# codelion/adaptive-classifier

Measured on NVIDIA H100. Metric: queries/sec predict() bert-base 128-tok, 1M x 768 prototypes, higher is better.
Workload: dtype f16

## Files before the change

### adaptive_classifier_b200/csrc/api.cu

```cuda
#include "common.cuh"
#include <cstdarg>
#include <cudaTypedefs.h>
#include <atomic>
#include <mutex>
#include <vector>

namespace ac {

static thread_local char g_err[512] = "";

void set_error(const char *fmt, ...) {
    va_list ap;
    va_start(ap, fmt);
    vsnprintf(g_err, sizeof(g_err), fmt, ap);
    va_end(ap);
}

int check_cuda(cudaError_t e, const char *what) {
    if (e == cudaSuccess) return AC_OK;
    set_error("CUDA error %d (%s) at %s", static_cast<int>(e), cudaGetErrorString(e), what);
    return AC_E_CUDA;
}

static std::atomic<long long> g_launches{0};
void count_launch() { g_launches.fetch_add(1, std::memory_order_relaxed); }
void count_launch_n(long long n) { g_launches.fetch_add(n, std::memory_order_relaxed); }
long long launch_count_now() { return g_launches.load(std::memory_order_relaxed); }

struct ProfSlot { cudaEvent_t a, b; int cls; double flops, bytes; };
static bool g_prof_on = false;
bool prof_is_on() { return g_prof_on; }
static std::vector<ProfSlot> g_prof_slots;
static size_t g_prof_used = 0;
static double g_prof_ms[PROF_NUM], g_prof_flops[PROF_NUM], g_prof_bytes[PROF_NUM];
static long long g_prof_n[PROF_NUM];

static void prof_harvest() {
    cudaDeviceSynchronize();
    for (size_t i = 0; i < g_prof_used; ++i) {
        float ms = 0.f;
        if (cudaEventElapsedTime(&ms, g_prof_slots[i].a, g_prof_slots[i].b) == cudaSuccess) {
            const int c = g_prof_slots[i].cls;
            g_prof_ms[c] += ms; g_prof_flops[c] += g_prof_slots[i].flops; g_prof_bytes[c] += g_prof_slots[i].bytes;
            g_prof_n[c] += 1;
        }
    }
    g_prof_used = 0;
}

int prof_begin(int cls, double flops, double bytes, cudaStream_t s) {
    if (!g_prof_on) return -1;
    if (g_prof_used == g_prof_slots.size()) {
        if (g_prof_slots.size() >= 8192) {
            prof_harvest();
        } else {
            ProfSlot p{};
            if (cudaEventCreate(&p.a) != cudaSuccess || cudaEventCreate(&p.b) != cudaSuccess) return -1;
            g_prof_slots.push_back(p);
        }
    }
    ProfSlot &p = g_prof_slots[g_prof_used];
    p.cls = cls; p.flops = flops; p.bytes = bytes;
    cudaEventRecord(p.a, s);
    return static_cast<int>(g_prof_used++);
}
void prof_end(int slot, cudaStream_t s) {
    if (slot < 0) return;
    cudaEventRecord(g_prof_slots[slot].b, s);
}

int sm_count() {
    static int n = 0;
    if (n == 0) {
        int dev = 0;
        if (cudaGetDevice(&dev) != cudaSuccess) return 132;
        if (cudaDeviceGetAttribute(&n, cudaDevAttrMultiProcessorCount, dev) != cudaSuccess || n <= 0) n = 132;
    }
    return n;
}

int make_tmap_2d(CUtensorMap *out, const void *gptr, int elem_bytes, uint64_t rows, uint64_t cols,
                 uint64_t row_stride_bytes, uint32_t box_rows, uint32_t box_cols) {
    static PFN_cuTensorMapEncodeTiled_v12000 encode = nullptr;
    static std::once_flag once;
    std::call_once(once, [] {
        void *fn = nullptr;
        cudaDriverEntryPointQueryResult qres;
        if (cudaGetDriverEntryPoint("cuTensorMapEncodeTiled", &fn, cudaEnableDefault, &qres) == cudaSuccess &&
            qres == cudaDriverEntryPointSuccess)
            encode = reinterpret_cast<PFN_cuTensorMapEncodeTiled_v12000>(fn);
    });
    if (!encode) {
        set_error("cuTensorMapEncodeTiled entry point not available (no CUDA driver?)");
        return AC_E_CUDA;
    }
    AC_REQUIRE((reinterpret_cast<uintptr_t>(gptr) & 15) == 0 && row_stride_bytes % 16 == 0,
               "make_tmap_2d: base pointer and row stride must be 16-byte aligned");
    AC_REQUIRE(box_cols * static_cast<uint32_t>(elem_bytes) == 128 && box_rows <= 256,
               "make_tmap_2d: box must be 128 bytes wide and <= 256 rows");
    const CUtensorMapDataType dt = (elem_bytes == 4) ? CU_TENSOR_MAP_DATA_TYPE_FLOAT32 : CU_TENSOR_MAP_DATA_TYPE_FLOAT16;
    cuuint64_t gdim[2] = {cols, rows};
    cuuint64_t gstride[1] = {row_stride_bytes};
    cuuint32_t box[2] = {box_cols, box_rows};
    cuuint32_t estr[2] = {1, 1};
    CUresult r = encode(out, dt, 2, const_cast<void *>(gptr), gdim, gstride, box, estr, CU_TENSOR_MAP_INTERLEAVE_NONE,
                        CU_TENSOR_MAP_SWIZZLE_128B, CU_TENSOR_MAP_L2_PROMOTION_L2_256B,
                        CU_TENSOR_MAP_FLOAT_OOB_FILL_NONE);
    if (r != CUDA_SUCCESS) {
        set_error("cuTensorMapEncodeTiled failed with CUresult %d (rows=%llu cols=%llu)", static_cast<int>(r),
                  static_cast<unsigned long long>(rows), static_cast<unsigned long long>(cols));
        return AC_E_CUDA;
    }
    return AC_OK;
}

int launch_knn_dist_exact(const float *Q, const float *P, int nq, int64_t N, int D, float *Dout, cudaStream_t stream);
int launch_knn_rerank(const float *Q, const float *P, int B, int64_t N, int D, int kc, const int32_t *cand, float *out_d,
                      int64_t *out_i, int64_t row_offset, cudaStream_t stream);
size_t topk_select_workspace(int B, int64_t L, int k);
int topk_select(const float *d, const int64_t *idx, int B, int64_t L, int64_t in_stride, int64_t id_offset, int k,
                float *out_d, int64_t *out_i, void *ws, size_t ws_bytes, cudaStream_t stream, const float *row_gate = nullptr);
size_t knn_tc_workspace(int B, int64_t N, int D, int k);
int knn_tc_search(const float *Q, const float *P, const float *p_sqnorm, const void *p_half, int B, int64_t N, int D, int k,
                  float *out_d, int64_t *out_i, int64_t row_offset, void *ws, size_t ws_bytes, int32_t *stats, cudaStream_t stream);

static int exact_query_block(int B, int64_t N) {
    const int64_t budget = 256ll << 20;
    int64_t qb = budget / (4 * (N > 0 ? N : 1));
    if (qb < 1) qb = 1;
    if (qb > B) qb = B;
    if (qb > 64) qb = 64;
    return static_cast<int>(qb);
}

static size_t knn_exact_workspace(int B, int64_t N, int k) {
    const int qb = exact_query_block(B, N);
    return align_up(static_cast<size_t>(qb) * N * sizeof(float), 256) + topk_select_workspace(qb, N, k) + 256;
}

static int knn_exact(const float *Q, const float *P, int B, int64_t N, int D, int k, float *out_d, int64_t *out_i,
                     int64_t row_offset, void *ws, size_t ws_bytes, cudaStream_t s) {
    const int qb = exact_query_block(B, N);
    const size_t dist_bytes = align_up(static_cast<size_t>(qb) * N * sizeof(float), 256);
    if (dist_bytes > ws_bytes) { set_error("ac_knn_l2_topk: workspace too small"); return AC_E_WORKSPACE; }
    float *dist = static_cast<float *>(ws);
    uint8_t *sel_ws = static_cast<uint8_t *>(ws) + dist_bytes;
    const size_t sel_bytes = ws_bytes - dist_bytes;
    for (int b0 = 0; b0 < B; b0 += qb) {
        const int nb = (B - b0 < qb) ? B - b0 : qb;
        int rc = launch_knn_dist_exact(Q + static_cast<int64_t>(b0) * D, P, nb, N, D, dist, s);
        if (rc) return rc;
        rc = topk_select(dist, nullptr, nb, N, N, row_offset, k, out_d + static_cast<int64_t>(b0) * k,
                         out_i + static_cast<int64_t>(b0) * k, sel_ws, sel_bytes, s);
        if (rc) return rc;
    }
    return AC_OK;
}

static int resolve_algo(int algo, int B, int64_t N, int D, int k) {
    if (algo != AC_KNN_AUTO) return algo;
    if (B >= 16 && k <= AC_KNN_TENSOR_MAX_K && N >= 4096 && N >= 8ll * k && D % 32 == 0) return AC_KNN_TENSOR;
    return AC_KNN_EXACT;
}

}

using namespace ac;

extern "C" int ac_version(void) { return 1; }
extern "C" long long ac_launch_count(void) { return g_launches.load(); }
extern "C" int ac_profile_enable(int on) {
    if (on && !g_prof_on) {
        for (int c = 0; c < PROF_NUM; ++c) { g_prof_ms[c] = g_prof_flops[c] = g_prof_bytes[c] = 0; g_prof_n[c] = 0; }
        g_prof_used = 0;
    }
    if (!on && g_prof_on) prof_harvest();
    g_prof_on = on != 0;
    return AC_OK;
}
extern "C" int ac_profile_read(int cls, double *ms, double *flops, double *bytes, long long *launches) {
    AC_REQUIRE(cls >= 0 && cls < PROF_NUM, "ac_profile_read: bad class");
    prof_harvest();
    if (ms) *ms = g_prof_ms[cls];
    if (flops) *flops = g_prof_flops[cls];
    if (bytes) *bytes = g_prof_bytes[cls];
    if (launches) *launches = g_prof_n[cls];
    return AC_OK;
}
extern "C" const char *ac_last_error(void) { return g_err; }

extern "C" int ac_device_check(void) {
    int n = 0;
    cudaError_t e = cudaGetDeviceCount(&n);
    if (e != cudaSuccess || n <= 0) {
        set_error("no CUDA device visible (%s); this library has no CPU fallback", cudaGetErrorString(e));
        return AC_E_CUDA;
    }
    int dev = 0, major = 0, minor = 0;
    AC_CUDA(cudaGetDevice(&dev));
    AC_CUDA(cudaDeviceGetAttribute(&major, cudaDevAttrComputeCapabilityMajor, dev));
    AC_CUDA(cudaDeviceGetAttribute(&minor, cudaDevAttrComputeCapabilityMinor, dev));
    if (major != 9 || minor != 0) {
        set_error("device compute capability %d.%d is not sm_90 (H100); kernels are sm_90a only", major, minor);
        return AC_E_CUDA;
    }
    return AC_OK;
}

extern "C" int ac_knn_workspace_bytes(int B, int64_t N, int D, int k, int algo, size_t *bytes) {
    AC_REQUIRE(bytes && B >= 0 && N >= 0 && D > 0 && k >= 1, "ac_knn_workspace_bytes: bad arguments");
    AC_REQUIRE(k <= AC_KNN_MAX_K, "ac_knn_workspace_bytes: k=%d > %d", k, AC_KNN_MAX_K);
    const int a = resolve_algo(algo, B, N, D, k);
    size_t need = knn_exact_workspace(B, N, k);
    if (a == AC_KNN_TENSOR) need += knn_tc_workspace(B, N, D, k);
    *bytes = need + 256;
    return AC_OK;
}

extern "C" int ac_knn_l2_topk(const float *Q, const float *P, const float *p_sqnorm, const void *p_half, int B, int64_t N,
                              int D, int k, float *out_d, int64_t *out_i, int64_t row_offset, void *workspace,
                              size_t workspace_bytes, int algo, int32_t *stats, ac_stream_t stream) {
    AC_REQUIRE(Q && out_d && out_i && B >= 0 && N >= 0 && D > 0, "ac_knn_l2_topk: bad arguments");
    AC_REQUIRE(k >= 1 && k <= AC_KNN_MAX_K, "ac_knn_l2_topk: k=%d outside [1,%d]", k, AC_KNN_MAX_K);
    AC_REQUIRE(N == 0 || P, "ac_knn_l2_topk: null index");
    AC_REQUIRE(N < (1ll << 31), "ac_knn_l2_topk: shards are limited to 2^31-1 rows");
    if (B == 0) return AC_OK;
    cudaStream_t s = static_cast<cudaStream_t>(stream);
    const int a = resolve_algo(algo, B, N, D, k);
    uint8_t *ws = static_cast<uint8_t *>(workspace);
    ws = reinterpret_cast<uint8_t *>(align_up(reinterpret_cast<uintptr_t>(ws), 256));
    const size_t slack = static_cast<size_t>(ws - static_cast<uint8_t *>(workspace));
    AC_REQUIRE(workspace && workspace_bytes > slack, "ac_knn_l2_topk: null/empty workspace");
    const size_t avail = workspace_bytes - slack;
    if (a == AC_KNN_TENSOR) {
        AC_REQUIRE(k <= AC_KNN_TENSOR_MAX_K && D % 32 == 0, "ac_knn_l2_topk: tensor path needs k <= %d and D %% 32 == 0", AC_KNN_TENSOR_MAX_K);
        AC_REQUIRE(!p_half || D % 64 == 0, "ac_knn_l2_topk: the fp16 shadow path needs D %% 64 == 0");
        return knn_tc_search(Q, P, p_sqnorm, p_half, B, N, D, k, out_d, out_i, row_offset, ws, avail, stats, s);
    }
    return knn_exact(Q, P, B, N, D, k, out_d, out_i, row_offset, ws, avail, s);
}

namespace ac {
int knn_exact_subset(const float *Q, const float *P, int B, int64_t N, int D, int k, float *out_d, int64_t *out_i,
                     int64_t row_offset, void *ws, size_t ws_bytes, cudaStream_t s) {
    return knn_exact(Q, P, B, N, D, k, out_d, out_i, row_offset, ws, ws_bytes, s);
}
size_t knn_exact_workspace_pub(int B, int64_t N, int k) { return knn_exact_workspace(B, N, k); }
}
```

### adaptive_classifier_b200/csrc/gemm_tc.cuh

```cuda
#pragma once
#include "common.cuh"

namespace ac {

constexpr int GEMM_BLOCK_M = 128;
constexpr int GEMM_BLOCK_N = 128;
constexpr int GEMM_BLOCK_K = 32;
constexpr int GEMM_KIND_TF32 = 0, GEMM_KIND_F16 = 1;
__host__ __device__ constexpr int gemm_block_k(int kind) { return kind == GEMM_KIND_F16 ? 64 : 32; }
constexpr int GEMM_STAGES = 4;
constexpr int GEMM_EPI_COLS = GEMM_BLOCK_N / 2;
constexpr int GEMM_EPI_WARPS = 8;
constexpr int GEMM_MMA_THREAD0 = 32 * GEMM_EPI_WARPS;
constexpr int GEMM_PRODUCER_THREAD = GEMM_MMA_THREAD0 + 128;
constexpr int GEMM_THREADS = GEMM_PRODUCER_THREAD + 128;
constexpr int GEMM_EPI_REGS = 160, GEMM_MMA_REGS = 160, GEMM_PRODUCER_REGS = 24;
static_assert(128 * GEMM_PRODUCER_REGS + 128 * GEMM_MMA_REGS + 256 * GEMM_EPI_REGS <= 65536, "register split exceeds the file");
constexpr int GEMM_A_STAGE_BYTES = GEMM_BLOCK_M * 128;
constexpr int GEMM_B_STAGE_BYTES = GEMM_BLOCK_N * 128;
constexpr int GEMM_STAGE_BYTES = GEMM_A_STAGE_BYTES + GEMM_B_STAGE_BYTES;
constexpr int GEMM_ACC_LD = GEMM_BLOCK_N + 4;
constexpr int GEMM_ACC_BYTES = GEMM_BLOCK_M * GEMM_ACC_LD * 4;
constexpr int GEMM_EPI_STAGE_ROW_BYTES = 80;
constexpr int GEMM_EPI_STAGE_BYTES = 32 * GEMM_EPI_STAGE_ROW_BYTES;
constexpr int GEMM_SMEM_BYTES = GEMM_STAGES * GEMM_STAGE_BYTES + GEMM_ACC_BYTES + GEMM_EPI_WARPS * GEMM_EPI_STAGE_BYTES +
                                1024  + 256 ;
static_assert(GEMM_SMEM_BYTES <= 227 * 1024, "stage ring + accumulator tile do not fit");

#ifndef AC_MBAR_WATCHDOG
#define AC_MBAR_WATCHDOG 1
#endif

__device__ __forceinline__ void mbar_wait_guarded(uint64_t *bar, uint32_t parity) {
#if AC_MBAR_WATCHDOG
    uint32_t spins = 0;
    while (!mbar_try_wait(bar, parity)) {
        if (++spins > (1u << 26)) __trap();
    }
#else
    mbar_wait(bar, parity);
#endif
}

struct GemmTileInfo {
    int m0, n0;
    int tile_iter;
};

__device__ __forceinline__ int gemm_epi_chalf() { return ((threadIdx.x >> 5) >> 1) & 1; }

template <class Epi, bool kMFastest = false, int kKind = GEMM_KIND_TF32>
__global__ void __launch_bounds__(GEMM_THREADS, 1)
gemm_tc_kernel(const __grid_constant__ CUtensorMap tmap_a, const __grid_constant__ CUtensorMap tmap_b,
               int M, int N, int K, Epi epi) {
    if (epi.skip_kernel()) return;
    extern __shared__ uint8_t smem_raw[];
    uint8_t *smem = reinterpret_cast<uint8_t *>((reinterpret_cast<uintptr_t>(smem_raw) + 1023) & ~uintptr_t(1023));
    uint8_t *smem_a = smem;
    uint8_t *smem_b = smem + GEMM_STAGES * GEMM_A_STAGE_BYTES;
    float *acc_tile = reinterpret_cast<float *>(smem + GEMM_STAGES * GEMM_STAGE_BYTES);
    uint8_t *epi_stage = smem + GEMM_STAGES * GEMM_STAGE_BYTES + GEMM_ACC_BYTES;
    uint64_t *bars = reinterpret_cast<uint64_t *>(epi_stage + GEMM_EPI_WARPS * GEMM_EPI_STAGE_BYTES);
    uint64_t *full_bar = bars;
    uint64_t *empty_bar = bars + GEMM_STAGES;
    uint64_t *acc_full = bars + 2 * GEMM_STAGES;
    uint64_t *acc_empty = acc_full + 1;

    const int warp = threadIdx.x >> 5;
    const int lane = threadIdx.x & 31;
    const int tiles_m = (M + GEMM_BLOCK_M - 1) / GEMM_BLOCK_M;
    const int tiles_n = (N + GEMM_BLOCK_N - 1) / GEMM_BLOCK_N;
    const int num_tiles = tiles_m * tiles_n;
    constexpr int BK = gemm_block_k(kKind);
    const int num_kb = (K + BK - 1) / BK;
    const int my_tiles = (num_tiles - static_cast<int>(blockIdx.x) + static_cast<int>(gridDim.x) - 1) / static_cast<int>(gridDim.x);

    if (threadIdx.x == GEMM_PRODUCER_THREAD) {
        tma_prefetch_desc(&tmap_a);
        tma_prefetch_desc(&tmap_b);
        for (int s = 0; s < GEMM_STAGES; ++s) {
            mbar_init(&full_bar[s], 1);
            mbar_init(&empty_bar[s], 4);
        }
        mbar_init(acc_full, 128);
        mbar_init(acc_empty, 32 * GEMM_EPI_WARPS);
        fence_mbar_init();
    }
    __syncthreads();

    if (threadIdx.x >= GEMM_PRODUCER_THREAD) {
        setmaxnreg_dec<GEMM_PRODUCER_REGS>();
        if (threadIdx.x == GEMM_PRODUCER_THREAD) {
            int stage = 0;
            uint32_t phase = 0;
            for (int tile = blockIdx.x; tile < num_tiles; tile += gridDim.x) {
                const int m0 = (kMFastest ? tile % tiles_m : tile / tiles_n) * GEMM_BLOCK_M;
                const int n0 = (kMFastest ? tile / tiles_m : tile % tiles_n) * GEMM_BLOCK_N;
                for (int kb = 0; kb < num_kb; ++kb) {
                    mbar_wait_guarded(&empty_bar[stage], phase ^ 1);
                    mbar_arrive_expect_tx(&full_bar[stage], GEMM_STAGE_BYTES);
                    tma_load_2d(smem_a + stage * GEMM_A_STAGE_BYTES, &tmap_a, &full_bar[stage], kb * BK, m0);
                    tma_load_2d(smem_b + stage * GEMM_B_STAGE_BYTES, &tmap_b, &full_bar[stage], kb * BK, n0);
                    if (++stage == GEMM_STAGES) { stage = 0; phase ^= 1; }
                }
            }
        }
        return;
    }

    if (threadIdx.x >= GEMM_MMA_THREAD0) {
        setmaxnreg_inc<GEMM_MMA_REGS>();
        const uint64_t a_desc0 = wgmma_desc_sw128(smem_u32(smem_a));
        const uint64_t b_desc0 = wgmma_desc_sw128(smem_u32(smem_b));
        int stage = 0;
        uint32_t phase = 0;
        for (int it = 0; it < my_tiles; ++it) {
            float acc0[64], acc1[64];
#pragma unroll
            for (int j = 0; j < 64; ++j) { acc0[j] = 0.f; acc1[j] = 0.f; }
            int prev_stage = -1;
            for (int kb = 0; kb < num_kb; ++kb) {
                mbar_wait_guarded(&full_bar[stage], phase);
                const uint64_t a_desc = a_desc0 + stage * (GEMM_A_STAGE_BYTES >> 4);
                const uint64_t b_desc = b_desc0 + stage * (GEMM_B_STAGE_BYTES >> 4);
                wgmma_fence();
#pragma unroll
                for (int k = 0; k < 4; ++k) {
                    if (kKind == GEMM_KIND_F16) {
                        wgmma_m64n128_f16(acc0, a_desc + 2 * k, b_desc + 2 * k, 1u);
                        wgmma_m64n128_f16(acc1, a_desc + 512 + 2 * k, b_desc + 2 * k, 1u);
                    } else {
                        wgmma_m64n128_tf32(acc0, a_desc + 2 * k, b_desc + 2 * k, 1u);
                        wgmma_m64n128_tf32(acc1, a_desc + 512 + 2 * k, b_desc + 2 * k, 1u);
                    }
                }
                wgmma_commit();
                wgmma_wait<1>();
                __syncwarp();
                if (prev_stage >= 0 && lane == 0) mbar_arrive(&empty_bar[prev_stage]);
                prev_stage = stage;
                if (++stage == GEMM_STAGES) { stage = 0; phase ^= 1; }
            }
            wgmma_wait<0>();
            __syncwarp();
            if (lane == 0) mbar_arrive(&empty_bar[prev_stage]);

            mbar_wait_guarded(acc_empty, (it & 1) ^ 1);
            wgmma_store_acc(acc0, acc_tile, GEMM_ACC_LD);
            wgmma_store_acc(acc1, acc_tile + 64 * GEMM_ACC_LD, GEMM_ACC_LD);
            mbar_arrive(acc_full);
        }
        return;
    }

    setmaxnreg_inc<GEMM_EPI_REGS>();
    const int wg = warp >> 2;
    const int q = 2 * wg + (warp & 1);
    const int chalf = gemm_epi_chalf();
    typename Epi::State est;
    epi.begin_cta(est, q, lane);
    const float *acc_row = acc_tile + (q * 32 + lane) * GEMM_ACC_LD;
    for (int it = 0; it < my_tiles; ++it) {
        const int tile = static_cast<int>(blockIdx.x) + it * static_cast<int>(gridDim.x);
        GemmTileInfo ti;
        ti.m0 = (kMFastest ? tile % tiles_m : tile / tiles_n) * GEMM_BLOCK_M;
        ti.n0 = (kMFastest ? tile / tiles_m : tile % tiles_n) * GEMM_BLOCK_N;
        ti.tile_iter = it;
        const int row = ti.m0 + q * 32 + lane;
        const int c_lo = chalf * GEMM_EPI_COLS;
        constexpr int kDist = Epi::kPrefetchDist, kBufs = kDist + 1, kChunks = GEMM_EPI_COLS / 32;
#pragma unroll
        for (int d = 0; d < kDist; ++d)
            if (d < kChunks) epi.prefetch(est, ti, row, ti.n0 + c_lo + 32 * d, lane, d % kBufs);

        mbar_wait_guarded(acc_full, it & 1);
#pragma unroll (Epi::kUnrollChunks)
        for (int ci = 0; ci < kChunks; ++ci) {
            const int c = c_lo + 32 * ci;
            if (ci + kDist < kChunks) epi.prefetch(est, ti, row, ti.n0 + c + 32 * kDist, lane, (ci + kDist) % kBufs);
            float v[32];
            acc_row_ld32(acc_row + c, v);
            epi.tile(est, ti, row, ti.n0 + c, v, epi_stage + warp * GEMM_EPI_STAGE_BYTES, lane, ci % kBufs, acc_row + c);
        }
        mbar_arrive(acc_empty);
    }
    epi.end_cta(est, q, lane);
}

template <class Epi, bool kMFastest = false, int kKind = GEMM_KIND_TF32>
int launch_gemm_tc(const CUtensorMap &ta, const CUtensorMap &tb, int M, int N, int K, const Epi &epi,
                   cudaStream_t stream, int max_ctas = 0, int prof_cls = PROF_GEMM_LINEAR, double prof_bytes = 0.0) {
    auto kern = gemm_tc_kernel<Epi, kMFastest, kKind>;
    static bool attr_set[64] = {};
    int dev = 0;
    AC_CUDA(cudaGetDevice(&dev));
    if (dev < 0 || dev >= 64 || !attr_set[dev]) {
        AC_CUDA(cudaFuncSetAttribute(kern, cudaFuncAttributeMaxDynamicSharedMemorySize, GEMM_SMEM_BYTES));
        if (dev >= 0 && dev < 64) attr_set[dev] = true;
    }
    const int tiles = ((M + GEMM_BLOCK_M - 1) / GEMM_BLOCK_M) * ((N + GEMM_BLOCK_N - 1) / GEMM_BLOCK_N);
    int ctas = sm_count();
    if (max_ctas > 0 && max_ctas < ctas) ctas = max_ctas;
    if (tiles < ctas) ctas = tiles;
    if (ctas <= 0) return AC_OK;
    const int slot = prof_begin(prof_cls, 2.0 * M * static_cast<double>(N) * K, prof_bytes, stream);
    kern<<<ctas, GEMM_THREADS, GEMM_SMEM_BYTES, stream>>>(ta, tb, M, N, K, epi);
    prof_end(slot, stream);
    AC_LAUNCH_CHECK();
    return AC_OK;
}

}
```

Measured before the change: 13640.

## Split accumulator handoff per half and overlap next tile's MMA with stores

The MMA consumer loop now commits the two 64-row wgmma chains as separate groups and releases each smem stage one step later. Each accumulator half gets its own full/empty barrier pair, with each epilogue warpgroup waiting only on its half. The first k-block of the next tile is issued while the previous tile's halves are stored, so tensor cores stay busy during the accumulator handoff. Compile-time-disabled phase timing instrumentation is also added; the risks are extra register pressure and subtle barrier-phase bugs.

```diff
diff --git a/adaptive_classifier_b200/csrc/api.cu b/adaptive_classifier_b200/csrc/api.cu
--- a/adaptive_classifier_b200/csrc/api.cu
+++ b/adaptive_classifier_b200/csrc/api.cu
@@ -1,4 +1,7 @@
 #include "common.cuh"
+#if AC_GEMM_PHASE_TIMES
+#include "gemm_tc.cuh"
+#endif
 #include <cstdarg>
 #include <cudaTypedefs.h>
 #include <atomic>
@@ -114,6 +117,11 @@
     return AC_OK;
 }
 
+#if AC_GEMM_PHASE_TIMES
+unsigned long long *g_gemm_phase_dev = nullptr;
+int g_gemm_phase_launches = 0;
+#endif
+
 int launch_knn_dist_exact(const float *Q, const float *P, int nq, int64_t N, int D, float *Dout, cudaStream_t stream);
 int launch_knn_rerank(const float *Q, const float *P, int B, int64_t N, int D, int kc, const int32_t *cand, float *out_d,
                       int64_t *out_i, int64_t row_offset, cudaStream_t stream);
@@ -188,6 +196,24 @@
     return AC_OK;
 }
 extern "C" const char *ac_last_error(void) { return g_err; }
+
+#if AC_GEMM_PHASE_TIMES
+extern "C" int ac_gemm_phase_times(int enable, unsigned long long *out, int *n_launches) {
+    const size_t bytes = sizeof(unsigned long long) * GEMM_PHASE_MAX_LAUNCHES * GEMM_PHASE_CTAS * GEMM_PH_SLOTS;
+    AC_CUDA(cudaDeviceSynchronize());
+    if (n_launches) *n_launches = g_gemm_phase_launches;
+    if (out && g_gemm_phase_dev) AC_CUDA(cudaMemcpy(out, g_gemm_phase_dev, bytes, cudaMemcpyDeviceToHost));
+    if (enable) {
+        if (!g_gemm_phase_dev) AC_CUDA(cudaMalloc(reinterpret_cast<void **>(&g_gemm_phase_dev), bytes));
+        AC_CUDA(cudaMemset(g_gemm_phase_dev, 0, bytes));
+    } else if (g_gemm_phase_dev) {
+        AC_CUDA(cudaFree(g_gemm_phase_dev));
+        g_gemm_phase_dev = nullptr;
+    }
+    g_gemm_phase_launches = 0;
+    return AC_OK;
+}
+#endif
 
 extern "C" int ac_device_check(void) {
     int n = 0;
diff --git a/adaptive_classifier_b200/csrc/gemm_tc.cuh b/adaptive_classifier_b200/csrc/gemm_tc.cuh
--- a/adaptive_classifier_b200/csrc/gemm_tc.cuh
+++ b/adaptive_classifier_b200/csrc/gemm_tc.cuh
@@ -42,6 +42,68 @@
 #endif
 }
 
+#ifndef AC_GEMM_PHASE_TIMES
+#define AC_GEMM_PHASE_TIMES 0
+#endif
+#if AC_GEMM_PHASE_TIMES
+enum {
+    GEMM_PH_TILES = 0,
+    GEMM_PH_FIRST_KB,
+    GEMM_PH_MAINLOOP,
+    GEMM_PH_ACC_EMPTY0,
+    GEMM_PH_STORE0,
+    GEMM_PH_DRAIN1,
+    GEMM_PH_ACC_EMPTY1,
+    GEMM_PH_STORE1,
+    GEMM_PH_CYCLES,
+    GEMM_PH_NS,
+    GEMM_PH_SLOTS = 16
+};
+constexpr int GEMM_PHASE_CTAS = 4, GEMM_PHASE_MAX_LAUNCHES = 256;
+extern unsigned long long *g_gemm_phase_dev;
+extern int g_gemm_phase_launches;
+static __device__ unsigned long long *g_gemm_phase_rec;
+
+__device__ __forceinline__ unsigned long long gemm_clock() {
+    unsigned long long t;
+    asm volatile("mov.u64 %0, %%clock64;" : "=l"(t)::"memory");
+    return t;
+}
+__device__ __forceinline__ unsigned long long gemm_globaltimer() {
+    unsigned long long t;
+    asm volatile("mov.u64 %0, %%globaltimer;" : "=l"(t)::"memory");
+    return t;
+}
+__device__ __forceinline__ void gemm_phase_stamp(unsigned long long *sm, int slot) {
+    asm volatile(
+        "{\n\t"
+        ".reg .pred p;\n\t"
+        ".reg .u64 t, a, b;\n\t"
+        "setp.eq.u32 p, %0, %1;\n\t"
+        "@p mov.u64 t, %%clock64;\n\t"
+        "@p ld.shared.u64 a, [%2];\n\t"
+        "@p ld.shared.u64 b, [%3];\n\t"
+        "@p sub.u64 a, t, a;\n\t"
+        "@p add.u64 b, b, a;\n\t"
+        "@p st.shared.u64 [%3], b;\n\t"
+        "@p st.shared.u64 [%2], t;\n\t"
+        "}" ::"r"(static_cast<uint32_t>(threadIdx.x)), "n"(GEMM_MMA_THREAD0), "r"(smem_u32(sm)), "r"(smem_u32(sm + slot))
+        : "memory");
+}
+#define AC_GEMM_STAMP(slot) gemm_phase_stamp(ph_smem, slot)
+#else
+#define AC_GEMM_STAMP(slot) do {} while (0)
+#endif
+
+template <int kKind>
+__device__ __forceinline__ void gemm_chain(float (&acc)[64], uint64_t a_desc, uint64_t b_desc) {
+#pragma unroll
+    for (int k = 0; k < 4; ++k) {
+        if (kKind == GEMM_KIND_F16) wgmma_m64n128_f16(acc, a_desc + 2 * k, b_desc + 2 * k, 1u);
+        else wgmma_m64n128_tf32(acc, a_desc + 2 * k, b_desc + 2 * k, 1u);
+    }
+}
+
 struct GemmTileInfo {
     int m0, n0;
     int tile_iter;
@@ -64,7 +126,10 @@
     uint64_t *full_bar = bars;
     uint64_t *empty_bar = bars + GEMM_STAGES;
     uint64_t *acc_full = bars + 2 * GEMM_STAGES;
-    uint64_t *acc_empty = acc_full + 1;
+    uint64_t *acc_empty = acc_full + 2;
+#if AC_GEMM_PHASE_TIMES
+    __shared__ unsigned long long ph_smem[GEMM_PH_SLOTS];
+#endif
 
     const int warp = threadIdx.x >> 5;
     const int lane = threadIdx.x & 31;
@@ -82,8 +147,10 @@
             mbar_init(&full_bar[s], 1);
             mbar_init(&empty_bar[s], 4);
         }
-        mbar_init(acc_full, 128);
-        mbar_init(acc_empty, 32 * GEMM_EPI_WARPS);
+        for (int h = 0; h < 2; ++h) {
+            mbar_init(&acc_full[h], 128);
+            mbar_init(&acc_empty[h], 128);
+        }
         fence_mbar_init();
     }
     __syncthreads();
@@ -114,42 +181,83 @@
         const uint64_t b_desc0 = wgmma_desc_sw128(smem_u32(smem_b));
         int stage = 0;
         uint32_t phase = 0;
-        for (int it = 0; it < my_tiles; ++it) {
-            float acc0[64], acc1[64];
-#pragma unroll
-            for (int j = 0; j < 64; ++j) { acc0[j] = 0.f; acc1[j] = 0.f; }
-            int prev_stage = -1;
-            for (int kb = 0; kb < num_kb; ++kb) {
+#if AC_GEMM_PHASE_TIMES
+        if (threadIdx.x == GEMM_MMA_THREAD0) {
+            for (int s = 1; s < GEMM_PH_SLOTS; ++s) ph_smem[s] = 0;
+            ph_smem[GEMM_PH_NS] = gemm_globaltimer();
+            ph_smem[0] = ph_smem[GEMM_PH_CYCLES] = gemm_clock();
+        }
+#endif
+        if (my_tiles == 0) return;
+        float acc0[64], acc1[64];
+#pragma unroll
+        for (int j = 0; j < 64; ++j) { acc0[j] = 0.f; acc1[j] = 0.f; }
+        int pending = stage;
+        mbar_wait_guarded(&full_bar[stage], phase);
+        AC_GEMM_STAMP(GEMM_PH_FIRST_KB);
+        wgmma_fence();
+        gemm_chain<kKind>(acc0, a_desc0, b_desc0);
+        wgmma_commit();
+        gemm_chain<kKind>(acc1, a_desc0 + 512, b_desc0);
+        wgmma_commit();
+        if (++stage == GEMM_STAGES) { stage = 0; phase ^= 1; }
+        for (int it = 0;; ++it) {
+            for (int kb = 1; kb < num_kb; ++kb) {
                 mbar_wait_guarded(&full_bar[stage], phase);
                 const uint64_t a_desc = a_desc0 + stage * (GEMM_A_STAGE_BYTES >> 4);
                 const uint64_t b_desc = b_desc0 + stage * (GEMM_B_STAGE_BYTES >> 4);
                 wgmma_fence();
-#pragma unroll
-                for (int k = 0; k < 4; ++k) {
-                    if (kKind == GEMM_KIND_F16) {
-                        wgmma_m64n128_f16(acc0, a_desc + 2 * k, b_desc + 2 * k, 1u);
-                        wgmma_m64n128_f16(acc1, a_desc + 512 + 2 * k, b_desc + 2 * k, 1u);
-                    } else {
-                        wgmma_m64n128_tf32(acc0, a_desc + 2 * k, b_desc + 2 * k, 1u);
-                        wgmma_m64n128_tf32(acc1, a_desc + 512 + 2 * k, b_desc + 2 * k, 1u);
-                    }
-                }
+                gemm_chain<kKind>(acc0, a_desc, b_desc);
                 wgmma_commit();
-                wgmma_wait<1>();
+                gemm_chain<kKind>(acc1, a_desc + 512, b_desc);
+                wgmma_commit();
+                wgmma_wait<2>();
                 __syncwarp();
-                if (prev_stage >= 0 && lane == 0) mbar_arrive(&empty_bar[prev_stage]);
-                prev_stage = stage;
+                if (lane == 0) mbar_arrive(&empty_bar[pending]);
+                pending = stage;
                 if (++stage == GEMM_STAGES) { stage = 0; phase ^= 1; }
             }
-            wgmma_wait<0>();
+            wgmma_wait<1>();
+            AC_GEMM_STAMP(GEMM_PH_MAINLOOP);
+            mbar_wait_guarded(&acc_empty[0], (it & 1) ^ 1);
+            AC_GEMM_STAMP(GEMM_PH_ACC_EMPTY0);
+            wgmma_store_acc(acc0, acc_tile, GEMM_ACC_LD);
+            AC_GEMM_STAMP(GEMM_PH_STORE0);
+            mbar_arrive(&acc_full[0]);
+            if (it + 1 == my_tiles) break;
+#pragma unroll
+            for (int j = 0; j < 64; ++j) acc0[j] = 0.f;
+            mbar_wait_guarded(&full_bar[stage], phase);
+            AC_GEMM_STAMP(GEMM_PH_FIRST_KB);
+            wgmma_fence();
+            gemm_chain<kKind>(acc0, a_desc0 + stage * (GEMM_A_STAGE_BYTES >> 4), b_desc0 + stage * (GEMM_B_STAGE_BYTES >> 4));
+            wgmma_commit();
+            wgmma_wait<1>();
+            AC_GEMM_STAMP(GEMM_PH_DRAIN1);
             __syncwarp();
-            if (lane == 0) mbar_arrive(&empty_bar[prev_stage]);
-
-            mbar_wait_guarded(acc_empty, (it & 1) ^ 1);
-            wgmma_store_acc(acc0, acc_tile, GEMM_ACC_LD);
+            if (lane == 0) mbar_arrive(&empty_bar[pending]);
+            mbar_wait_guarded(&acc_empty[1], (it & 1) ^ 1);
+            AC_GEMM_STAMP(GEMM_PH_ACC_EMPTY1);
             wgmma_store_acc(acc1, acc_tile + 64 * GEMM_ACC_LD, GEMM_ACC_LD);
-            mbar_arrive(acc_full);
-        }
+            AC_GEMM_STAMP(GEMM_PH_STORE1);
+            mbar_arrive(&acc_full[1]);
+#pragma unroll
+            for (int j = 0; j < 64; ++j) acc1[j] = 0.f;
+            wgmma_fence();
+            gemm_chain<kKind>(acc1, a_desc0 + stage * (GEMM_A_STAGE_BYTES >> 4) + 512, b_desc0 + stage * (GEMM_B_STAGE_BYTES >> 4));
+            wgmma_commit();
+            pending = stage;
+            if (++stage == GEMM_STAGES) { stage = 0; phase ^= 1; }
+        }
+        wgmma_wait<0>();
+        AC_GEMM_STAMP(GEMM_PH_DRAIN1);
+        __syncwarp();
+        if (lane == 0) mbar_arrive(&empty_bar[pending]);
+        mbar_wait_guarded(&acc_empty[1], ((my_tiles - 1) & 1) ^ 1);
+        AC_GEMM_STAMP(GEMM_PH_ACC_EMPTY1);
+        wgmma_store_acc(acc1, acc_tile + 64 * GEMM_ACC_LD, GEMM_ACC_LD);
+        AC_GEMM_STAMP(GEMM_PH_STORE1);
+        mbar_arrive(&acc_full[1]);
         return;
     }
 
@@ -173,7 +281,7 @@
         for (int d = 0; d < kDist; ++d)
             if (d < kChunks) epi.prefetch(est, ti, row, ti.n0 + c_lo + 32 * d, lane, d % kBufs);
 
-        mbar_wait_guarded(acc_full, it & 1);
+        mbar_wait_guarded(&acc_full[wg], it & 1);
 #pragma unroll (Epi::kUnrollChunks)
         for (int ci = 0; ci < kChunks; ++ci) {
             const int c = c_lo + 32 * ci;
@@ -182,9 +290,18 @@
             acc_row_ld32(acc_row + c, v);
             epi.tile(est, ti, row, ti.n0 + c, v, epi_stage + warp * GEMM_EPI_STAGE_BYTES, lane, ci % kBufs, acc_row + c);
         }
-        mbar_arrive(acc_empty);
+        mbar_arrive(&acc_empty[wg]);
     }
     epi.end_cta(est, q, lane);
+#if AC_GEMM_PHASE_TIMES
+    unsigned long long *rec = g_gemm_phase_rec;
+    if (rec && threadIdx.x == 128 && blockIdx.x < GEMM_PHASE_CTAS && my_tiles > 0) {
+        ph_smem[GEMM_PH_CYCLES] = gemm_clock() - ph_smem[GEMM_PH_CYCLES];
+        ph_smem[GEMM_PH_NS] = gemm_globaltimer() - ph_smem[GEMM_PH_NS];
+        ph_smem[GEMM_PH_TILES] = my_tiles;
+        for (int s = 0; s < GEMM_PH_SLOTS; ++s) rec[blockIdx.x * GEMM_PH_SLOTS + s] = ph_smem[s];
+    }
+#endif
 }
 
 template <class Epi, bool kMFastest = false, int kKind = GEMM_KIND_TF32>
@@ -204,6 +321,12 @@
     if (tiles < ctas) ctas = tiles;
     if (ctas <= 0) return AC_OK;
     const int slot = prof_begin(prof_cls, 2.0 * M * static_cast<double>(N) * K, prof_bytes, stream);
+#if AC_GEMM_PHASE_TIMES
+    unsigned long long *ph = nullptr;
+    if (g_gemm_phase_dev && g_gemm_phase_launches < GEMM_PHASE_MAX_LAUNCHES)
+        ph = g_gemm_phase_dev + static_cast<size_t>(g_gemm_phase_launches++) * GEMM_PHASE_CTAS * GEMM_PH_SLOTS;
+    AC_CUDA(cudaMemcpyToSymbolAsync(g_gemm_phase_rec, &ph, sizeof(ph), 0, cudaMemcpyHostToDevice, stream));
+#endif
     kern<<<ctas, GEMM_THREADS, GEMM_SMEM_BYTES, stream>>>(ta, tb, M, N, K, epi);
     prof_end(slot, stream);
     AC_LAUNCH_CHECK();
```

New measurement: 13850, median of 6. About the same (+1.5%).
